# nsbuitrago/parasail-rs

Hardware: AMD Instinct MI355X
Metric: GCUPS (cell updates/s) local-affine SW, 1M 150x150 pairs, 1/2/4/8 GPUs (higher is better)
Workload: dtype int16

## Files before the change

parasail-rs_amd/csrc/pmx_pk16.h:

```cpp
#pragma once
#include <hip/hip_runtime.h>

constexpr int PK16_LO = 1024;
constexpr int PK16_HI = 31743;
constexpr int PK16_SW_BIAS = 2048;
constexpr int PK16_SW_BIAS2 = (PK16_SW_BIAS << 16) | PK16_SW_BIAS;
#define PK16_RERUN_LIMIT(maxs) (PK16_HI + 1 - ((maxs) > 0 ? (maxs) : 0))

typedef short v2s __attribute__((ext_vector_type(2)));
typedef unsigned short v2us __attribute__((ext_vector_type(2)));
typedef _Float16 v2h __attribute__((ext_vector_type(2)));

#define PK(x)  __builtin_bit_cast(v2s, (int)(x))
#define I32(x) __builtin_bit_cast(int, (x))


__device__ __forceinline__ v2s pk_max3(v2s a, v2s b, v2s c)
{
    const v2h r = __builtin_elementwise_maximum(__builtin_elementwise_maximum(__builtin_bit_cast(v2h, a), __builtin_bit_cast(v2h, b)),
                                                __builtin_bit_cast(v2h, c));
    return __builtin_bit_cast(v2s, r);
}
__device__ __forceinline__ int pk_max3(int a, int b, int c)
{
    const v2h r = __builtin_elementwise_maximum(__builtin_elementwise_maximum(__builtin_bit_cast(v2h, a), __builtin_bit_cast(v2h, b)),
                                                __builtin_bit_cast(v2h, c));
    return __builtin_bit_cast(int, r);
}
__device__ __forceinline__ v2s pk_max3_asm(v2s a, v2s b, v2s c)
{
    int r;
    asm("v_pk_maximum3_f16 %0, %1, %2, %3" : "=v"(r) : "v"(I32(a)), "v"(I32(b)), "v"(I32(c)));
    return PK(r);
}

__device__ __forceinline__ v2s pk_subus(v2s a, v2s b)
{
    return __builtin_bit_cast(v2s, __builtin_elementwise_sub_sat(__builtin_bit_cast(v2us, a), __builtin_bit_cast(v2us, b)));
}
__device__ __forceinline__ int pk_subus(int a, int b)
{
    return __builtin_bit_cast(int, __builtin_elementwise_sub_sat(__builtin_bit_cast(v2us, a), __builtin_bit_cast(v2us, b)));
}

__device__ __forceinline__ int pk_lt(v2s a, v2s b) { const v2s sh = {15, 15}; return I32((a - b) >> sh); }
__device__ __forceinline__ int pk_lt(int a, int b) { return pk_lt(PK(a), PK(b)); }

__device__ __forceinline__ int bfi(int m, int a, int b)
{
    int r;
    asm("v_bfi_b32 %0, %1, %2, %3" : "=v"(r) : "v"(m), "v"(a), "v"(b));
    return r;
}
__device__ __forceinline__ int bfi_sgpr(int m, int a, int b)
{
    int r;
    asm("v_bfi_b32 %0, %1, %2, %3" : "=v"(r) : "s"(m), "v"(a), "v"(b));
    return r;
}


__device__ __forceinline__ unsigned add_u16(unsigned a, unsigned b) { unsigned r; asm("v_add_u16_e32 %0, %1, %2" : "=v"(r) : "v"(a), "v"(b)); return r; }
__device__ __forceinline__ unsigned sub_u16(unsigned a, unsigned b) { unsigned r; asm("v_sub_u16_e32 %0, %1, %2" : "=v"(r) : "v"(a), "v"(b)); return r; }
__device__ __forceinline__ unsigned max_u16(unsigned a, unsigned b) { unsigned r; asm("v_max_u16_e32 %0, %1, %2" : "=v"(r) : "v"(a), "v"(b)); return r; }


template <int G>
__device__ __forceinline__ int lane_prev(int old, int x)
{
    if (G <= 16) return __builtin_amdgcn_update_dpp(old, x, 0x111 , 0xF, 0xF, false);
    return __builtin_amdgcn_update_dpp(old, x, 0x138 , 0xF, 0xF, false);
}
template <int G>
__device__ __forceinline__ int lane_prev(int x) { return lane_prev<G>(x, x); }

template <int G, bool IL = false>
__device__ __forceinline__ int group_shift_up(int x, int neutral, int g)
{
    if (G == 1) return neutral;
    if (IL) return __builtin_amdgcn_update_dpp(neutral, x, 0x112 , 0xF, 0xF, false);
    const int r = lane_prev<G>(neutral, x);
    return (G == 16 || G == 64) ? r : (g == 0 ? neutral : r);
}

template <int G>
__device__ __forceinline__ int lane_next(int x)
{
    if (G <= 16) return __builtin_amdgcn_update_dpp(x, x, 0x101 , 0xF, 0xF, false);
    return __builtin_amdgcn_update_dpp(x, x, 0x130 , 0xF, 0xF, false);
}
__device__ __forceinline__ int lane_next_untied(int x) { return __builtin_amdgcn_update_dpp(0, x, 0x130 , 0xF, 0xF, true); }
```

parasail-rs_amd/csrc/pmx_sw16.hip:

```cpp
#include "pmx_common.h"
#include "pmx_switches.h"
#include "pmx_pk16.h"
#include <cstdlib>

__device__ __forceinline__ v2s pk_adds(v2s a, v2s b) { return __builtin_elementwise_add_sat(a, b); }
__device__ __forceinline__ v2s pk_subs(v2s a, v2s b) { return __builtin_elementwise_sub_sat(a, b); }
__device__ __forceinline__ v2s pk_max(v2s a, v2s b) { return __builtin_elementwise_max(a, b); }

#ifndef PMX_SHARE_PERIOD
#define PMX_SHARE_PERIOD 16
#endif
#define FLOOR2 0x80008000

template <int G, int R, int VAR>
__global__ __launch_bounds__(64, (VAR == 6 && R <= 20) ? 4 : 1)
void pmx_sw16_kernel(const uint8_t *__restrict__ qbuf, const int64_t *__restrict__ qoff,
                     const uint8_t *__restrict__ rbuf, const int64_t *__restrict__ roff,
                     long long n, const int16_t *__restrict__ gmat, const uint8_t *__restrict__ gmap,
                     int msize, int open, int ext, int RP ,
                     int q_shared ,
                     int limit ,
                     const unsigned *__restrict__ perm,
                     const int *__restrict__ n_dev ,
                     unsigned *__restrict__ retry_list, int *__restrict__ retry_count ,
                     int sat_above ,
                     uint32_t *__restrict__ tbuf, int Tmax ,
                     pmx_record_t *__restrict__ out)
{
    if (n_dev) n = *n_dev;
    if ((long long)blockIdx.x * (2 * (64 / G)) >= n) return;
    constexpr bool M3 = VAR >= 1;
    constexpr bool V2 = VAR >= 2;
    constexpr bool PT = VAR == 6;
    constexpr bool TR = VAR == 7;
    static_assert(!TR || R == 16, "trace: four packed planes of 4 rows");
    constexpr bool FETCH = VAR == 8;
    constexpr bool U8 = VAR == 3 || VAR == 5 || PT || TR || FETCH;
    constexpr bool SK = VAR >= 4;
    constexpr int EB = U8 ? 1 : 2;
    constexpr int WR = U8 ? 4 : 2;
    constexpr int RS = (R + WR - 1) / WR * WR;
    constexpr int QP = G * RS;
    constexpr int QP2 = QP / 2;
    constexpr int SLOTS = 64 / G;
    constexpr int NP = 2 * SLOTS;
    extern __shared__ __attribute__((aligned(16))) unsigned char lds[];

    const int lane = threadIdx.x;
    constexpr bool IL = G == 8 && VAR != 7;
    const int g = IL ? (lane % 16) / 2 : lane % G;
    const int slot = IL ? (lane / 16) * 2 + (lane & 1) : lane / G;
    const int PROF_STRIDE = PT ? 0 : msize * QP * EB;

    int16_t *prof = reinterpret_cast<int16_t *>(lds);
    unsigned char *rsym = lds + (PT ? 0 : NP * PROF_STRIDE + QP * EB);
    int16_t *mat = reinterpret_cast<int16_t *>(rsym + (FETCH ? 0 : NP * RP));
    unsigned char *map = reinterpret_cast<unsigned char *>(mat + msize * msize);
    long long *ptab = reinterpret_cast<long long *>(map + 256 + ((8 - ((msize * msize * 2) & 7)) & 7));

    int *tabs = reinterpret_cast<int *>(ptab + 5 * NP);
    constexpr int QS = (G * R + 3) / 4 * 4;
    unsigned char *qsym = reinterpret_cast<unsigned char *>(tabs + 8);

    const long long pair0 = (long long)blockIdx.x * NP;

    for (int i = lane; i < msize * msize; i += 64) mat[i] = gmat[i];
    for (int i = lane; i < 256; i += 64) map[i] = gmap[i];
    if (lane < NP) {
        long long pos = pair0 + lane; if (pos >= n) pos = n - 1;
        const long long pi = perm ? (long long)perm[pos] : pos;
        const long long qb = q_shared ? 0 : qoff[pi], rb = roff[pi];
        ptab[5 * lane + 0] = qb;
        ptab[5 * lane + 1] = q_shared ? q_shared : (qoff[pi + 1] - qb);
        ptab[5 * lane + 2] = rb;
        ptab[5 * lane + 3] = roff[pi + 1] - rb;
        ptab[5 * lane + 4] = (pair0 + lane < n) ? pi : -1;
    }
    __syncthreads();
    const uint8_t *qbase = qbuf;
    const uint8_t *rbase = rbuf;

    int max_rlen = 0;
#pragma unroll
    for (int p = 0; p < NP; ++p) max_rlen = max(max_rlen, (int)ptab[5 * p + 3]);
    constexpr int UB = NP < 8 ? NP : 8;
    for (int p0 = 0; p0 < (FETCH ? 0 : NP); p0 += UB) {
        for (int j0 = 0; j0 < RP; j0 += 64) {
            const int j = j0 + lane, jr = j - (G - 1);
            unsigned char raw[UB]; bool ok[UB];
#pragma unroll
            for (int u = 0; u < UB; ++u) {
                const int p = p0 + u;
                ok[u] = jr >= 0 && jr < (int)ptab[5 * p + 3];
                raw[u] = ok[u] ? rbase[ptab[5 * p + 2] + jr] : (unsigned char)0;
            }
            if (j < RP) {
#pragma unroll
                for (int u = 0; u < UB; ++u) {
                    const int p = p0 + u;
                    rsym[p * RP + j] = ok[u] ? map[raw[u]] : (unsigned char)(PT ? msize : (NP - p) * msize);
                }
            }
        }
    }

    if (PT) {
        for (int p0 = 0; p0 < NP; p0 += UB) {
            for (int j0 = 0; j0 < QS; j0 += 64) {
                const int j = j0 + lane;
                unsigned char raw[UB]; bool ok[UB];
#pragma unroll
                for (int u = 0; u < UB; ++u) {
                    const int p = p0 + u;
                    ok[u] = j < (int)ptab[5 * p + 1];
                    raw[u] = ok[u] ? qbase[ptab[5 * p + 0] + j] : (unsigned char)0;
                }
                if (j < QS) {
#pragma unroll
                    for (int u = 0; u < UB; ++u) qsym[(p0 + u) * QS + j] = ok[u] ? map[raw[u]] : (unsigned char)0xFF;
                }
            }
        }
    }

    constexpr int QITEMS = PT ? 0 : (NP * QP2 + 63) / 64;
    constexpr int QB = QITEMS < 5 ? (QITEMS < 1 ? 1 : QITEMS) : 5;
    for (int it0 = 0; it0 < QITEMS; it0 += QB) {
        unsigned char r0[QB], r1[QB]; bool v0[QB], v1[QB];
#pragma unroll
        for (int u = 0; u < QB; ++u) {
            const int item = (it0 + u) * 64 + lane;
            const int p = min(item / QP2, NP - 1), rp = item - p * QP2;
            const int ql = (int)ptab[5 * p + 1];
            const uint8_t *qp = qbase + ptab[5 * p + 0];
            const int p0 = 2 * rp, p1 = 2 * rp + 1;
            const int k0 = p0 % RS, k1 = p1 % RS;
            const int row0 = (p0 / RS) * R + k0, row1 = (p1 / RS) * R + k1;
            v0[u] = item < NP * QP2 && k0 < R && row0 < ql; v1[u] = item < NP * QP2 && k1 < R && row1 < ql;
            r0[u] = v0[u] ? qp[row0] : (unsigned char)0;
            r1[u] = v1[u] ? qp[row1] : (unsigned char)0;
        }
#pragma unroll
        for (int u = 0; u < QB; ++u) {
            const int item = (it0 + u) * 64 + lane;
            if (it0 + u < QITEMS && item < NP * QP2) {
                const int p = item / QP2, rp = item - p * QP2;
                const int q0 = v0[u] ? map[r0[u]] : -1;
                const int q1 = v1[u] ? map[r1[u]] : -1;
                for (int sym = 0; sym < msize; ++sym) {
                    const int s0 = ((q0 < 0) ? 0 : mat[q0 * msize + sym]) + (V2 ? open : 0);
                    const int s1 = ((q1 < 0) ? 0 : mat[q1 * msize + sym]) + (V2 ? open : 0);
                    if (U8) {
                        reinterpret_cast<unsigned short *>(lds + p * PROF_STRIDE + sym * QP)[rp] =
                            (unsigned short)((s0 & 0xFF) | ((s1 & 0xFF) << 8));
                    } else {
                        int *pp = reinterpret_cast<int *>(prof) + p * (PROF_STRIDE / 4) + rp;
                        pp[sym * QP2] = (s0 & 0xFFFF) | (s1 << 16);
                    }
                }
            }
        }
    }
    if (!PT) {
        for (int idx = lane; idx < QP * EB / 4; idx += 64)
            reinterpret_cast<int *>(lds + NP * PROF_STRIDE)[idx] = V2 ? 0 : FLOOR2;
    }
    int sel[R];
    int wild = 0;
    if (PT) {
        if (lane <= msize) {
            int v = 0;
            if (lane < msize)
                for (int k = 0; k < 4 && k < msize; ++k) v |= ((mat[k * msize + lane] + open) & 0xFF) << (8 * k);
            tabs[lane] = v;
        }
    }
    __syncthreads();
    if (PT) {
        const unsigned char *qa = qsym + (2 * slot) * QS + g * R, *qb = qa + QS;
#pragma unroll
        for (int k = 0; k < R; ++k) {
            const int ca = qa[k], cb = qb[k];
            wild |= ((ca >= 4 && ca != 0xFF) ? 1 : 0) | ((cb >= 4 && cb != 0xFF) ? 2 : 0);
            sel[k] = (ca < 4 ? ca : 0x0C) | 0x0C00 | ((cb < 4 ? 4 + cb : 0x0C) << 16) | 0x0C000000;
        }
        asm volatile("" : "+v"(wild));
    }
    __syncthreads();

    const int pA = 2 * slot, pB = 2 * slot + 1;
    const unsigned char *profA = lds + pA * PROF_STRIDE + g * (RS * EB);
    const unsigned char *profB = lds + pB * PROF_STRIDE + g * (RS * EB);
    const unsigned char *rsA = rsym + pA * RP + (G - 1) - g;
    const unsigned char *rsB = rsym + pB * RP + (G - 1) - g;
    const int SYMSTRIDE = QP * EB;

    const v2s vOpen = PK((open & 0xFFFF) | (open << 16));
    const v2s vExt = PK((ext & 0xFFFF) | (ext << 16));
    constexpr int ZERO2 = M3 ? PK16_SW_BIAS2 : FLOOR2;
    const v2s vZero = PK(ZERO2);

    v2s HA[R], HB[R], E[R], Hsave[R];
    const int skew0 = SK ? (((G - g) * ext) & 0xFFFF) * 0x00010001 : 0;
    const v2s vC = PK(I32(vOpen) - I32(vExt));
    const v2s vInitH = V2 ? PK(ZERO2 - I32(vOpen) + skew0) : vZero;
#pragma unroll
    for (int k = 0; k < R; ++k) { HA[k] = vInitH; HB[k] = vInitH; E[k] = V2 ? vInitH : (M3 ? PK(0) : vZero); Hsave[k] = vZero; }
    v2s best = PK(ZERO2 + skew0 - (SK ? I32(vC) : 0));
    int bestcol = g * 0x00010001;
    int vprev = 0, fake = 0;
    int Zv = ZERO2 + skew0 + I32(vExt);
    const int HNEUTRAL = V2 ? ZERO2 - I32(vOpen) : ZERO2;
    int Hout = SK ? Zv - I32(vExt) - I32(vOpen) : HNEUTRAL, Fout = SK ? Zv - I32(vExt) : ZERO2;
    v2s diag0 = PK(SK ? I32(vInitH) : HNEUTRAL);

    auto load_scores = [&](int symA, int symB, int (&wa)[RS / WR], int (&wb)[RS / WR]) {
        if (PT) { wa[0] = tabs[symA]; wb[0] = tabs[symB]; return; }
        const int *sa = reinterpret_cast<const int *>(profA + symA * SYMSTRIDE);
        const int *sb = reinterpret_cast<const int *>(profB + symB * SYMSTRIDE);
#pragma unroll
        for (int k = 0; k < RS / WR; ++k) { wa[k] = sa[k]; wb[k] = sb[k]; }
    };
    const size_t t_ss = 4;
    uint32_t *tw = TR ? tbuf + ((size_t)blockIdx.x * Tmax) * 256 + (size_t)lane * Tmax * 4 : nullptr;
    auto push = [&](v2s &pl, v2s a, v2s b) {
        const v2us fifteen = {15, 15};
        const int bit = I32(__builtin_bit_cast(v2s, __builtin_bit_cast(v2us, a - b) >> fifteen));
        int r;
        asm("v_pk_mad_u16 %0, %1, %2, %3" : "=v"(r) : "v"(I32(pl)), "v"(0x00020002), "v"(bit));
        pl = PK(r);
    };
    auto step = [&](const v2s (&Hold)[R], v2s (&Hnew)[R], const int (&wa)[RS / WR], const int (&wb)[RS / WR], int t) {
        const int Hin = group_shift_up<G, IL>(Hout, SK ? Zv - I32(vOpen) : HNEUTRAL, g);
        const int Fin = group_shift_up<G, IL>(Fout, SK ? Zv : ZERO2, g);
        v2s F = PK(Fin);
        v2s colmax = SK ? PK(0) : vZero;
        v2s Hcur[R];
        v2s Tpre[R], Epre[R];
        v2s plane[TR ? R / 4 : 1];
        if (TR) {
#pragma unroll
            for (int x = 0; x < R / 4; ++x) plane[x] = PK(0);
        }
        if (V2) {
#pragma unroll
            for (int k = 0; k < R; ++k) {
                const v2s s = PT ? PK(__builtin_amdgcn_perm(wb[0], wa[0], (unsigned)sel[k]))
                            : U8 ? PK(__builtin_amdgcn_perm(wb[k / 4], wa[k / 4], 0x0C000C00u | (unsigned)(k & 3) | ((4u + (unsigned)(k & 3)) << 16)))
                               : PK(__builtin_amdgcn_perm(wb[k / 2], wa[k / 2], (k & 1) ? 0x07060302 : 0x05040100));
                const v2s d = (k == 0) ? diag0 : Hold[k - 1];
                Tpre[k] = PK(I32(d) + I32(s));
                if (!SK) Epre[k] = PK(I32(E[k]) - I32(vExt));
            }
            __builtin_amdgcn_sched_barrier(0);
        }
#pragma unroll
        for (int k = 0; k < R; ++k) {
            const v2s s = PT ? PK(__builtin_amdgcn_perm(wb[0], wa[0], (unsigned)sel[k]))
                        : U8 ? PK(__builtin_amdgcn_perm(wb[k / 4], wa[k / 4], 0x0C000C00u | (unsigned)(k & 3) | ((4u + (unsigned)(k & 3)) << 16)))
                               : PK(__builtin_amdgcn_perm(wb[k / 2], wa[k / 2], (k & 1) ? 0x07060302 : 0x05040100));
            const v2s d = (k == 0) ? diag0 : Hold[k - 1];
            v2s H;
            if (SK) {
                const v2s Fe = PK(I32(F) - I32(vExt));
                H = pk_max3(Tpre[k], E[k], Fe);
                const v2s X = PK(I32(H) - I32(vC));
                if (TR) {
                    push(plane[k / 4], Tpre[k], H);
                    push(plane[k / 4], Fe, H);
                    push(plane[k / 4], E[k], X);
                    push(plane[k / 4], Fe, X);
                }
                E[k] = pk_max3(E[k], X, X);
                F = pk_max3(Fe, X, PK(Zv));
                Hnew[k] = X;
                if (k & 1) colmax = pk_max3(colmax, Hnew[k - 1], X);
                else if (k == R - 1) colmax = pk_max3(colmax, X, best);
            } else if (V2) {
                H = pk_max3(Tpre[k], E[k], F);
                const v2s Ho = PK(I32(H) - I32(vOpen));
                E[k] = pk_max3(Epre[k], Ho, Ho);
                F = pk_max3(PK(I32(F) - I32(vExt)), Ho, vZero);
                Hnew[k] = Ho;
                Hcur[k] = H;
                if (k & 1) colmax = pk_max3(colmax, Hcur[k - 1], H);
                else if (k == R - 1) colmax = pk_max3(colmax, H, H);
            } else if (M3) {
                const v2s Tt = PK(I32(__builtin_bit_cast(v2us, d) + __builtin_bit_cast(v2us, s)));
                H = pk_max3(Tt, E[k], F);
                const v2s Ho = pk_subus(H, vOpen);
                E[k] = pk_max3(pk_subus(E[k], vExt), Ho, Ho);
                F = pk_max3(pk_subus(F, vExt), Ho, vZero);
                Hnew[k] = H;
                if (k & 1) colmax = pk_max3(colmax, Hnew[k - 1], H);
                else if (k == R - 1) colmax = pk_max3(colmax, H, H);
            } else {
                H = pk_adds(d, s);
                H = pk_max(H, E[k]);
                H = pk_max(H, F);
                const v2s Ho = pk_subs(H, vOpen);
                E[k] = pk_max(pk_subs(E[k], vExt), Ho);
                F = pk_max(pk_subs(F, vExt), Ho);
                Hnew[k] = H;
                colmax = pk_max(colmax, H);
            }
        }
        if (TR) {
            uint4 w;
            w.x = __builtin_amdgcn_perm(I32(plane[0]), I32(plane[1]), 0x00010405);
            w.y = __builtin_amdgcn_perm(I32(plane[2]), I32(plane[3]), 0x00010405);
            w.z = __builtin_amdgcn_perm(I32(plane[0]), I32(plane[1]), 0x02030607);
            w.w = __builtin_amdgcn_perm(I32(plane[2]), I32(plane[3]), 0x02030607);
            *reinterpret_cast<uint4 *>(tw + (size_t)t * t_ss) = w;
        }
        diag0 = PK(Hin);
        Hout = I32(Hnew[R - 1]);
        Fout = I32(F);
        constexpr bool FOLDED = SK && (R & 1);
        const v2s nb = FOLDED ? colmax : M3 ? pk_max3(best, colmax, colmax) : pk_max(best, colmax);
        int m;
        {
            const v2s dd = FOLDED ? (best - nb) : M3 ? (best - colmax) : pk_subs(best, colmax);
            const v2s sh = {15, 15};
            m = I32(dd >> sh);
        }
        if (__builtin_amdgcn_ballot_w64(m != 0) != 0) {
            asm("v_bfi_b32 %0, %1, %2, %3" : "=v"(bestcol) : "v"(m), "s"((t & 0xFFFF) * 0x00010001), "v"(bestcol));
            fake &= ~m;
#pragma unroll
            for (int k = 0; k < R; ++k) Hsave[k] = PK(bfi(m, I32((V2 && !SK) ? Hcur[k] : Hnew[k]), I32(Hsave[k])));
        }
        best = SK ? PK(I32(nb) + I32(vExt)) : nb;
        if (SK) Zv += I32(vExt);
    };

    const int T = max_rlen + G - 1;
    int w0a[RS / WR], w0b[RS / WR], w1a[RS / WR], w1b[RS / WR];
    const int rlA_ = (int)ptab[5 * pA + 3], rlB_ = (int)ptab[5 * pB + 3];
    const uint8_t *refA = rbase + ptab[5 * pA + 2], *refB = rbase + ptab[5 * pB + 2];
    auto fetch = [&](int x, int &ra, int &rb) {
        const int col = x - g;
        ra = (col >= 0 && col < rlA_) ? (int)refA[col] : -1;
        rb = (col >= 0 && col < rlB_) ? (int)refB[col] : -1;
    };
    auto symA_of = [&](int raw) -> int { return raw < 0 ? (NP - pA) * msize : (int)map[raw]; };
    auto symB_of = [&](int raw) -> int { return raw < 0 ? (NP - pB) * msize : (int)map[raw]; };
    int m2a = 0, m2b = 0, m3a = 0, m3b = 0, nsA, nsB;
    if (FETCH) {
        int r0a, r0b, r1a, r1b;
        fetch(0, r0a, r0b); fetch(1, r1a, r1b); fetch(2, m2a, m2b); fetch(3, m3a, m3b);
        load_scores(symA_of(r0a), symB_of(r0b), w0a, w0b);
        nsA = symA_of(r1a); nsB = symB_of(r1b);
    } else {
        load_scores(rsA[0], rsB[0], w0a, w0b);
        nsA = rsA[1]; nsB = rsB[1];
    }
    constexpr int SHP = PMX_SHARE_PERIOD > G ? PMX_SHARE_PERIOD : G;
    auto share_bound = [&]() {
        int v = I32(best) - skew0;
#pragma unroll
        for (int off = G / 2; off >= 1; off >>= 1) {
            const int o = __shfl_xor(v, (IL ? 2 : 1) * off, 64);
            v = pk_max3(v, o, o);
        }
        const int fresh = v - 0x00010001 + skew0;
        const int old = vprev ? vprev + ((SHP * ext) & 0xFFFF) * 0x00010001 + skew0 : 0;
        const v2s nbest = pk_max3(best, PK(fresh), PK(old));
        fake |= pk_lt(best, nbest);
        best = nbest;
        vprev = v;
    };
    for (int t = 0; t + 1 < T; t += 2) {
        if (SK && G > 1 && (t & (SHP - 1)) == 0 && t) share_bound();
        load_scores(nsA, nsB, w1a, w1b);
        if (FETCH) { nsA = symA_of(m2a); nsB = symB_of(m2b); fetch(t + 4, m2a, m2b); }
        else { nsA = rsA[t + 2]; nsB = rsB[t + 2]; }
        __builtin_amdgcn_sched_barrier(0);
        step(HA, HB, w0a, w0b, t);
        __builtin_amdgcn_sched_barrier(0);
        load_scores(nsA, nsB, w0a, w0b);
        if (FETCH) { nsA = symA_of(m3a); nsB = symB_of(m3b); fetch(t + 5, m3a, m3b); }
        else { nsA = rsA[t + 3]; nsB = rsB[t + 3]; }
        __builtin_amdgcn_sched_barrier(0);
        step(HB, HA, w1a, w1b, t + 1);
        __builtin_amdgcn_sched_barrier(0);
    }
    if (T & 1) step(HA, HB, w0a, w0b, T - 1);

    unsigned long long keyA, keyB;
    {
        const int bA = (short)(I32(best) & 0xFFFF), bB = (short)(I32(best) >> 16);
        const unsigned stA = bestcol & 0xFFFF, stB = (unsigned)bestcol >> 16;
        const unsigned cA = stA - g, cB = stB - g;
        const int tA = SK ? bA - (T - (int)stA) * ext : bA, tB = SK ? bB - (T - (int)stB) * ext : bB;
        int kA = 0, kB = 0;
#pragma unroll
        for (int k = R - 1; k >= 0; --k) {
            if ((short)(I32(Hsave[k]) & 0xFFFF) == tA) kA = k;
            if ((short)(I32(Hsave[k]) >> 16) == tB) kB = k;
        }
        const int unskew = SK ? (G - g + T) * ext - (open - ext) : 0;
        const unsigned sA = (unsigned)(bA - unskew - (M3 ? PK16_SW_BIAS : -32768)), sB = (unsigned)(bB - unskew - (M3 ? PK16_SW_BIAS : -32768));
        const unsigned rA = g * R + kA, rB = g * R + kB;
        keyA = ((unsigned long long)sA << 32) | ((0xFFFFu - cA) << 16) | (0xFFFFu - rA);
        keyB = ((unsigned long long)sB << 32) | ((0xFFFFu - cB) << 16) | (0xFFFFu - rB);
        if (fake & 0xFFFF) keyA = 0;
        if (fake >> 16) keyB = 0;
    }
#pragma unroll
    for (int off = G / 2; off >= 1; off >>= 1) {
        const int lo = IL ? 2 * off : off;
        const unsigned long long oa = __shfl_xor(keyA, lo, 64), ob = __shfl_xor(keyB, lo, 64);
        keyA = oa > keyA ? oa : keyA;
        keyB = ob > keyB ? ob : keyB;
        if (PT) wild |= __shfl_xor(wild, lo, 64);
    }
    if (g == 0) {
#pragma unroll
        for (int h = 0; h < 2; ++h) {
            const long long pi = ptab[5 * (2 * slot + h) + 4];
            if (pi >= 0) {
                const unsigned long long key = h ? keyB : keyA;
                pmx_record_t rec;
                rec.score = (int)(key >> 32);
                rec.end_ref = 0xFFFF - (int)((key >> 16) & 0xFFFF);
                rec.end_query = 0xFFFF - (int)(key & 0xFFFF);
                if (M3) rec.flags = (rec.score + PK16_SW_BIAS >= limit) ? PMX_FLAG_RERUN : 0;
                else rec.flags = rec.score > 32767 ? PMX_FLAG_SATURATED : 0;
                if (rec.score > sat_above) rec.flags |= PMX_FLAG_SATURATED;
                if (PT && ((wild >> h) & 1)) {
                    rec.flags = PMX_FLAG_RETRY16;
                    retry_list[atomicAdd(retry_count, 1)] = (unsigned)pi;
                }
                out[pi] = rec;
            }
        }
    }
}


template <int G, int R, int VAR>
static int launch_one(const PmxBatch &b, const PmxDevMatrix &m, int open, int ext,
                      pmx_record_t *d_out, hipStream_t stream, const int *n_dev = nullptr, uint32_t *tbuf = nullptr, int Tmax = 0)
{
    constexpr bool PT = VAR == 6;
    constexpr int EB = (VAR == 3 || VAR == 5 || VAR == 7 || VAR == 8 || PT) ? 1 : 2, WR = 4 / EB, RS = (R + WR - 1) / WR * WR;
    constexpr int QP = G * RS, NP = 2 * (64 / G);
    if (NP * m.msize > 255) return 1;
    const int RP = ((b.max_rlen + 2 * (G - 1) + 4 + 7) / 4) * 4;
    const size_t lds = (PT ? (size_t)NP * ((G * R + 3) / 4 * 4) : (size_t)NP * m.msize * QP * EB + (size_t)QP * EB) + (VAR == 8 ? 0 : (size_t)NP * RP) +
                       (size_t)m.msize * m.msize * 2 + 256 + 8 + (size_t)NP * 40 + 32;
    if (lds > 160 * 1024) return 1;
    { const int rc = pmx_ensure_lds_attr(reinterpret_cast<const void *>(&pmx_sw16_kernel<G, R, VAR>)); if (rc) return rc; }
    const long long blocks = (b.n + NP - 1) / NP;
    if (blocks <= 0) return 0;
    if (PT) {
        hipError_t e = hipMemsetAsync(b.retry_count, 0, sizeof(int), stream);
        if (e != hipSuccess) return -(int)e;
    }
    hipLaunchKernelGGL((pmx_sw16_kernel<G, R, VAR>), dim3((unsigned)blocks), dim3(64), lds, stream,
                       b.qbuf, b.qoff, b.rbuf, b.roff, (long long)b.n, m.scores, m.mapper,
                       m.msize, open, ext, RP, b.q_shared, PK16_RERUN_LIMIT(m.max) - (VAR >= 4 ? (b.max_rlen + 2 * G + 4) * ext : 0), b.perm,
                       n_dev, b.retry_list, b.retry_count, b.sat_above > 0 ? b.sat_above : 2147483647, tbuf, Tmax, d_out);
    hipError_t e = hipGetLastError();
    if (e != hipSuccess) return -(int)e;
    if (PT) {
        PmxBatch r = b;
        r.perm = b.retry_list;
        return launch_one<G, R, 5>(r, m, open, ext, d_out, stream, b.retry_count);
    }
    return 0;
}

static bool sw16_trace_ok(const PmxBatch &b, const PmxDevMatrix &m, int open, int ext)
{
    if (pmx_env("PMX_TRACE16_GEN1") || pmx_env("PMX_SW16_NO_SKEW") || pmx_env("PMX_SW16_NO_U8") || pmx_env("PMX_SW16_VARIANT")) return false;
    if (m.msize > PMX_MAX_FAST_MSIZE || open < ext || ext < 0 || open > 1024 || b.max_rlen > 30000 || b.q_shared || b.perm) return false;
    if (m.min < -1024 || m.max > 2048 || m.min + open < 0 || open + ext > 1024 || m.max + open > 255) return false;
    const long long feasible = (long long)(b.max_qlen < b.max_rlen ? b.max_qlen : b.max_rlen) * (m.max > 0 ? m.max : 0);
    return feasible + PK16_SW_BIAS < (long long)PK16_RERUN_LIMIT(m.max) - (long long)(b.max_rlen + 2 * 64 + 4) * ext;
}
int pmx_sw16_trace_plan(const PmxBatch &b, const PmxDevMatrix &m, int open, int ext, int *variant, int *Tmax, size_t *trace_bytes)
{
    if (!sw16_trace_ok(b, m, open, ext)) return 1;
    if (m.msize > 8 && m.msize < 32 && !pmx_env("PMX_SW16_NO_MATRIX_LOOKUP")) {
        int G = 0;
        for (int v = 1; v < 4 && !G; ++v) if (b.max_qlen <= (8 << v) * 16) { *variant = 4 + v; G = 8 << v; }
        if (!G) return 1;
        *Tmax = (b.max_rlen + G - 1 + 1 + 15) & ~15;
        *trace_bytes = (size_t)((b.n + 2 * (64 / G) - 1) / (2 * (64 / G))) * (size_t)*Tmax * 64 * 16;
        return 0;
    }
    int G = 0;
    for (int v = 0; v < 4 && !G; ++v) {
        const int g = 8 << v, np = 2 * (64 / g);
        const size_t lds = (size_t)np * m.msize * g * 16 + (size_t)g * 16 + (size_t)np * (b.max_rlen + 2 * g + 12) +
                           (size_t)m.msize * m.msize * 2 + 256 + 8 + (size_t)np * 40 + 32;
        if (b.max_qlen <= g * 16 && np * m.msize <= 255 && lds <= 160 * 1024) { *variant = v; G = g; }
    }
    if (!G) return 1;
    const int NP = 2 * (64 / G);
    *Tmax = (b.max_rlen + G - 1 + 15) & ~15;
    *trace_bytes = (size_t)((b.n + NP - 1) / NP) * (size_t)*Tmax * 64 * 16;
    return 0;
}
int pmx_launch_sw16_trace(int variant, const PmxBatch &b, const PmxDevMatrix &m, int open, int ext,
                          pmx_record_t *d_out, uint32_t *tbuf, int Tmax, hipStream_t stream)
{
    if (!sw16_trace_ok(b, m, open, ext)) return 1;
    if (variant >= 4) return pmx_launch_sw16m_trace(variant - 4, b, m, open, ext, d_out, tbuf, Tmax, stream);
    switch (variant) {
    case 0: return launch_one<8, 16, 7>(b, m, open, ext, d_out, stream, nullptr, tbuf, Tmax);
    case 1: return launch_one<16, 16, 7>(b, m, open, ext, d_out, stream, nullptr, tbuf, Tmax);
    case 2: return launch_one<32, 16, 7>(b, m, open, ext, d_out, stream, nullptr, tbuf, Tmax);
    case 3: return launch_one<64, 16, 7>(b, m, open, ext, d_out, stream, nullptr, tbuf, Tmax);
    }
    return 1;
}

int pmx_launch_sw16(const PmxBatch &b, const PmxDevMatrix &m, int open, int ext,
                    pmx_record_t *d_out, hipStream_t stream, const char **kernel_name)
{
    if (m.msize > PMX_MAX_FAST_MSIZE) return 1;
    if (open < 0 || ext < 0 || open > 32767 || ext > 32767) return 1;
    if (m.max > 32767 || m.min < -32767) return 1;
    if (b.max_rlen > 60000) return 1;
    const int q = b.max_qlen;
    const char *force = pmx_env("PMX_SW16_VARIANT");
    int var = 0;
    if (open <= 1024 && ext <= 1024 && m.min >= -1024 && m.max <= 2048) var = 1;
    if (var == 1 && m.min + open >= 0 && open + ext <= 1024) var = 2;
    if (force && atoi(force) < var) var = atoi(force);
    const bool u8ok = var == 2 && m.max + open <= 255 && !pmx_env("PMX_SW16_NO_U8");
    const long long feasible = (long long)(b.max_qlen < b.max_rlen ? b.max_qlen : b.max_rlen) * (m.max > 0 ? m.max : 0);
    const bool sk = var == 2 && open >= ext && !pmx_env("PMX_SW16_NO_SKEW") &&
                    feasible + PK16_SW_BIAS < (long long)PK16_RERUN_LIMIT(m.max) - (long long)(b.max_rlen + 2 * 64 + 4) * ext;
    const bool pt = sk && u8ok && m.msize <= 5 && b.retry_list && b.retry_count && !b.q_has_wildcard && !pmx_env("PMX_SW16_NO_PERMTABLE");
    if (b.q_shared && var == 2 && u8ok && sk && !pt) {
        const int rc = pmx_launch_sw16q(b, m, open, ext, d_out, stream, kernel_name);
        if (rc <= 0) return rc;
    }
    if (!b.q_shared && var == 2 && u8ok && sk && !pt && (m.msize > 8 || pmx_env("PMX_SW16_MATRIX_LOOKUP")) && b.n > 2048) {
        const int rc = pmx_launch_sw16m(b, m, open, ext, d_out, stream, kernel_name);
        if (rc <= 0) return rc;
    }
    const bool longref = b.max_rlen >= 1024 && !pmx_env("PMX_SW16_NO_FETCH");
#define TRY(GG, RR, NAME)                                                       \
    if (q <= (GG) * (RR)) {                                                     \
        constexpr int R4 = (RR);             \
        const bool u8 = u8ok;                                                   \
        int rc = pt ? launch_one<GG, RR, 6>(b, m, open, ext, d_out, stream)     \
               : (u8 && sk && longref) ? launch_one<GG, R4, 8>(b, m, open, ext, d_out, stream)  \
               : (u8 && sk) ? launch_one<GG, R4, 5>(b, m, open, ext, d_out, stream)  \
               : u8 ? launch_one<GG, R4, 3>(b, m, open, ext, d_out, stream)     \
               : (var == 2 && sk) ? launch_one<GG, RR, 4>(b, m, open, ext, d_out, stream)  \
               : var == 2 ? launch_one<GG, RR, 2>(b, m, open, ext, d_out, stream)  \
               : var == 1 ? launch_one<GG, RR, 1>(b, m, open, ext, d_out, stream)  \
                          : launch_one<GG, RR, 0>(b, m, open, ext, d_out, stream); \
        if (rc <= 0) { if (kernel_name) *kernel_name = pt ? NAME "/max3+vop2+skew+permtable" : var == 2 ? (sk ? ((u8 && longref) ? NAME "/max3+vop2+u8+skew+fetch" : NAME "/max3+vop2+skew") : NAME "/max3+vop2") : var == 1 ? NAME "/max3" : NAME; return rc; } \
    }
#define TRY8(RR)                                                                \
    if (u8ok && q <= 8 * (RR)) {                                                \
        int rc = pt ? launch_one<8, RR, 6>(b, m, open, ext, d_out, stream)      \
               : sk ? launch_one<8, RR, 5>(b, m, open, ext, d_out, stream) : launch_one<8, RR, 3>(b, m, open, ext, d_out, stream); \
        if (rc <= 0) { if (kernel_name) *kernel_name = pt ? "pmx_sw16_kernel<8," #RR ">/max3+vop2+skew+permtable" : sk ? "pmx_sw16_kernel<8," #RR ">/max3+vop2+u8+skew" : "pmx_sw16_kernel<8," #RR ">/max3+vop2+u8"; return rc; } \
    }
    if (b.n > 2048) { TRY8(7) TRY8(10) TRY8(13) TRY8(16) TRY8(19) TRY8(20) }
#undef TRY8
#define TRYLAT(RR)                                                              \
    if (u8ok && sk && !longref && b.n <= 64 && q <= 64 * (RR)) {                \
        const int rc = launch_one<64, RR, 5>(b, m, open, ext, d_out, stream);   \
        if (rc <= 0) { if (kernel_name) *kernel_name = "pmx_sw16_kernel<64," #RR ">/max3+vop2+u8+skew"; return rc; } \
    }
    TRYLAT(2) TRYLAT(3) TRYLAT(4) TRYLAT(8)
#undef TRYLAT
    TRY(16, 10, "pmx_sw16_kernel<16,10>")
    TRY(16, 16, "pmx_sw16_kernel<16,16>")
    TRY(32, 10, "pmx_sw16_kernel<32,10>")
    TRY(32, 16, "pmx_sw16_kernel<32,16>")
    TRY(64, 16, "pmx_sw16_kernel<64,16>")
    TRY(64, 32, "pmx_sw16_kernel<64,32>")
#undef TRY
    return 1;
}
```

Baseline: 8022.

## Interleave PT reference symbols, use DPP group max, and skip folded compare

For the packed-table (PT) variant, the score table moves to LDS address 0 and symbols are stored pre-multiplied by 4 with A/B pairs interleaved. This lets each step fetch both symbols from adjacent bytes through a running pointer and read the table by direct byte address. The shuffle-based group max reduction is replaced by DPP row operations, falling back to bpermute only across rows. For folded SK kernels the improvement mask is computed only after the ballot fires. The trip count is also made wave-uniform with readfirstlane. Together these aim to cut address arithmetic, LDS shuffles and VALU work in the inner loop, at the cost of a more complex LDS layout.

```diff
diff --git a/parasail-rs_amd/csrc/pmx_pk16.h b/parasail-rs_amd/csrc/pmx_pk16.h
--- a/parasail-rs_amd/csrc/pmx_pk16.h
+++ b/parasail-rs_amd/csrc/pmx_pk16.h
@@ -90,3 +90,25 @@
     return __builtin_amdgcn_update_dpp(x, x, 0x130 , 0xF, 0xF, false);
 }
 __device__ __forceinline__ int lane_next_untied(int x) { return __builtin_amdgcn_update_dpp(0, x, 0x130 , 0xF, 0xF, true); }
+
+template <int CTRL>
+__device__ __forceinline__ int row_dpp(int x) { return __builtin_amdgcn_update_dpp(0, x, CTRL, 0xF, 0xF, true); }
+
+template <int G, bool IL = false>
+__device__ __forceinline__ int group_max3(int v)
+{
+    if constexpr (IL || G >= 16) {
+        if (!IL) { const int o = row_dpp<0x121 >(v); v = pk_max3(v, o, o); }
+        { const int o = row_dpp<0x122 >(v); v = pk_max3(v, o, o); }
+        { const int o = row_dpp<0x124 >(v); v = pk_max3(v, o, o); }
+        { const int o = row_dpp<0x128 >(v); v = pk_max3(v, o, o); }
+    } else {
+        static_assert(G == 1 || G == 2 || G == 4 || G == 8, "adjacent groups inside a row");
+        if (G >= 2) { const int o = row_dpp<0xB1 >(v); v = pk_max3(v, o, o); }
+        if (G >= 4) { const int o = row_dpp<0x4E >(v); v = pk_max3(v, o, o); }
+        if (G >= 8) { const int o = row_dpp<0x141 >(v); v = pk_max3(v, o, o); }
+    }
+    if (G >= 32) { const int o = __builtin_amdgcn_ds_bpermute(((int)__lane_id() ^ 16) * 4, v); v = pk_max3(v, o, o); }
+    if (G >= 64) { const int o = __builtin_amdgcn_ds_bpermute(((int)__lane_id() ^ 32) * 4, v); v = pk_max3(v, o, o); }
+    return v;
+}
diff --git a/parasail-rs_amd/csrc/pmx_sw16.hip b/parasail-rs_amd/csrc/pmx_sw16.hip
--- a/parasail-rs_amd/csrc/pmx_sw16.hip
+++ b/parasail-rs_amd/csrc/pmx_sw16.hip
@@ -52,15 +52,17 @@
     const int slot = IL ? (lane / 16) * 2 + (lane & 1) : lane / G;
     const int PROF_STRIDE = PT ? 0 : msize * QP * EB;
 
+    constexpr int PT_TABS = 32;
     int16_t *prof = reinterpret_cast<int16_t *>(lds);
-    unsigned char *rsym = lds + (PT ? 0 : NP * PROF_STRIDE + QP * EB);
+    unsigned char *rsym = lds + (PT ? PT_TABS : NP * PROF_STRIDE + QP * EB);
     int16_t *mat = reinterpret_cast<int16_t *>(rsym + (FETCH ? 0 : NP * RP));
     unsigned char *map = reinterpret_cast<unsigned char *>(mat + msize * msize);
     long long *ptab = reinterpret_cast<long long *>(map + 256 + ((8 - ((msize * msize * 2) & 7)) & 7));
 
-    int *tabs = reinterpret_cast<int *>(ptab + 5 * NP);
+    typedef __attribute__((address_space(3))) int *lds_int;
+    auto tab_at = [](int byte) -> int { return *(lds_int)(uintptr_t)byte; };
     constexpr int QS = (G * R + 3) / 4 * 4;
-    unsigned char *qsym = reinterpret_cast<unsigned char *>(tabs + 8);
+    unsigned char *qsym = reinterpret_cast<unsigned char *>(ptab + 5 * NP);
 
     const long long pair0 = (long long)blockIdx.x * NP;
 
@@ -98,7 +100,10 @@
 #pragma unroll
                 for (int u = 0; u < UB; ++u) {
                     const int p = p0 + u;
-                    rsym[p * RP + j] = ok[u] ? map[raw[u]] : (unsigned char)(PT ? msize : (NP - p) * msize);
+                    if (PT)
+                        rsym[(p >> 1) * 2 * RP + 2 * j + (p & 1)] = (unsigned char)(4 * (ok[u] ? map[raw[u]] : msize));
+                    else
+                        rsym[p * RP + j] = ok[u] ? map[raw[u]] : (unsigned char)((NP - p) * msize);
                 }
             }
         }
@@ -172,7 +177,7 @@
             int v = 0;
             if (lane < msize)
                 for (int k = 0; k < 4 && k < msize; ++k) v |= ((mat[k * msize + lane] + open) & 0xFF) << (8 * k);
-            tabs[lane] = v;
+            ((lds_int)(uintptr_t)0)[lane] = v;
         }
     }
     __syncthreads();
@@ -191,8 +196,9 @@
     const int pA = 2 * slot, pB = 2 * slot + 1;
     const unsigned char *profA = lds + pA * PROF_STRIDE + g * (RS * EB);
     const unsigned char *profB = lds + pB * PROF_STRIDE + g * (RS * EB);
-    const unsigned char *rsA = rsym + pA * RP + (G - 1) - g;
-    const unsigned char *rsB = rsym + pB * RP + (G - 1) - g;
+    constexpr int SS = PT ? 2 : 1;
+    const unsigned char *rsA = PT ? rsym + slot * 2 * RP + 2 * ((G - 1) - g) : rsym + pA * RP + (G - 1) - g;
+    const unsigned char *rsB = PT ? rsA + 1 : rsym + pB * RP + (G - 1) - g;
     const int SYMSTRIDE = QP * EB;
 
     const v2s vOpen = PK((open & 0xFFFF) | (open << 16));
@@ -215,7 +221,7 @@
     v2s diag0 = PK(SK ? I32(vInitH) : HNEUTRAL);
 
     auto load_scores = [&](int symA, int symB, int (&wa)[RS / WR], int (&wb)[RS / WR]) {
-        if (PT) { wa[0] = tabs[symA]; wb[0] = tabs[symB]; return; }
+        if (PT) { wa[0] = tab_at(symA); wb[0] = tab_at(symB); return; }
         const int *sa = reinterpret_cast<const int *>(profA + symA * SYMSTRIDE);
         const int *sb = reinterpret_cast<const int *>(profB + symB * SYMSTRIDE);
 #pragma unroll
@@ -318,13 +324,14 @@
         Fout = I32(F);
         constexpr bool FOLDED = SK && (R & 1);
         const v2s nb = FOLDED ? colmax : M3 ? pk_max3(best, colmax, colmax) : pk_max(best, colmax);
-        int m;
-        {
+        auto improved = [&]() -> int {
             const v2s dd = FOLDED ? (best - nb) : M3 ? (best - colmax) : pk_subs(best, colmax);
             const v2s sh = {15, 15};
-            m = I32(dd >> sh);
-        }
-        if (__builtin_amdgcn_ballot_w64(m != 0) != 0) {
+            return I32(dd >> sh);
+        };
+        int m = FOLDED ? 0 : improved();
+        if (__builtin_amdgcn_ballot_w64(FOLDED ? I32(nb) != I32(best) : m != 0) != 0) {
+            if (FOLDED) m = improved();
             asm("v_bfi_b32 %0, %1, %2, %3" : "=v"(bestcol) : "v"(m), "s"((t & 0xFFFF) * 0x00010001), "v"(bestcol));
             fake &= ~m;
 #pragma unroll
@@ -334,7 +341,7 @@
         if (SK) Zv += I32(vExt);
     };
 
-    const int T = max_rlen + G - 1;
+    const int T = __builtin_amdgcn_readfirstlane(max_rlen) + G - 1;
     int w0a[RS / WR], w0b[RS / WR], w1a[RS / WR], w1b[RS / WR];
     const int rlA_ = (int)ptab[5 * pA + 3], rlB_ = (int)ptab[5 * pB + 3];
     const uint8_t *refA = rbase + ptab[5 * pA + 2], *refB = rbase + ptab[5 * pB + 2];
@@ -353,16 +360,11 @@
         nsA = symA_of(r1a); nsB = symB_of(r1b);
     } else {
         load_scores(rsA[0], rsB[0], w0a, w0b);
-        nsA = rsA[1]; nsB = rsB[1];
+        nsA = rsA[SS]; nsB = rsB[SS];
     }
     constexpr int SHP = PMX_SHARE_PERIOD > G ? PMX_SHARE_PERIOD : G;
     auto share_bound = [&]() {
-        int v = I32(best) - skew0;
-#pragma unroll
-        for (int off = G / 2; off >= 1; off >>= 1) {
-            const int o = __shfl_xor(v, (IL ? 2 : 1) * off, 64);
-            v = pk_max3(v, o, o);
-        }
+        const int v = group_max3<G, IL>(I32(best) - skew0);
         const int fresh = v - 0x00010001 + skew0;
         const int old = vprev ? vprev + ((SHP * ext) & 0xFFFF) * 0x00010001 + skew0 : 0;
         const v2s nbest = pk_max3(best, PK(fresh), PK(old));
@@ -370,16 +372,19 @@
         best = nbest;
         vprev = v;
     };
+    const unsigned char *rcur = rsA;
     for (int t = 0; t + 1 < T; t += 2) {
         if (SK && G > 1 && (t & (SHP - 1)) == 0 && t) share_bound();
         load_scores(nsA, nsB, w1a, w1b);
         if (FETCH) { nsA = symA_of(m2a); nsB = symB_of(m2b); fetch(t + 4, m2a, m2b); }
+        else if (PT) { nsA = rcur[2 * SS]; nsB = rcur[2 * SS + 1]; asm("" : "+v"(nsA), "+v"(nsB)); }
         else { nsA = rsA[t + 2]; nsB = rsB[t + 2]; }
         __builtin_amdgcn_sched_barrier(0);
         step(HA, HB, w0a, w0b, t);
         __builtin_amdgcn_sched_barrier(0);
         load_scores(nsA, nsB, w0a, w0b);
         if (FETCH) { nsA = symA_of(m3a); nsB = symB_of(m3b); fetch(t + 5, m3a, m3b); }
+        else if (PT) { nsA = rcur[3 * SS]; nsB = rcur[3 * SS + 1]; asm("" : "+v"(nsA), "+v"(nsB)); rcur += 2 * SS; }
         else { nsA = rsA[t + 3]; nsB = rsB[t + 3]; }
         __builtin_amdgcn_sched_barrier(0);
         step(HB, HA, w1a, w1b, t + 1);
```

After: 8240, median of 6. 2.7% higher.
